# ROCm/k8s-device-plugin

Measured on AMD Instinct MI355X. Metric: pod_admission_device_grants_per_s, higher is better.
Workload: dtype n/a; 1 GPU; model=stub-kubelet-pod-admission, devices_per_allocate=1, parallelism=node-local, server=native, sysfs=live, advertised_gpus=1, present_gpus=1, pinned_cpus=16

## Files before the change

### k8s_device_plugin_amd/native/fastserver.cpp

```cpp

#include <arpa/inet.h>
#include <errno.h>
#include <fcntl.h>
#include <poll.h>
#include <string.h>
#include <sys/socket.h>
#include <sys/un.h>
#include <unistd.h>

#include <algorithm>
#include <atomic>
#include <chrono>
#include <cstdint>
#include <map>
#include <memory>
#include <mutex>
#include <string>
#include <thread>
#include <unordered_map>
#include <vector>

#include <pybind11/pybind11.h>
#include <pybind11/stl.h>

#include "nghttp2_abi.h"
#include "pref_alloc.h"

namespace py = pybind11;
using prefalloc::AllocState;
using prefalloc::preferred_alloc;

namespace {


void put_varint(std::string &out, uint64_t v) {
    while (v >= 0x80) {
        out.push_back((char)(v | 0x80));
        v >>= 7;
    }
    out.push_back((char)v);
}

bool get_varint(const uint8_t *&p, const uint8_t *end, uint64_t &v) {
    v = 0;
    int shift = 0;
    while (p < end && shift < 64) {
        uint8_t b = *p++;
        v |= (uint64_t)(b & 0x7F) << shift;
        if (!(b & 0x80)) return true;
        shift += 7;
    }
    return false;
}

void put_len_delim(std::string &out, int field, const std::string &bytes) {
    put_varint(out, (uint64_t)(field << 3) | 2);
    put_varint(out, bytes.size());
    out += bytes;
}

template <typename F>
bool for_each_field(const uint8_t *p, const uint8_t *end, F cb) {
    while (p < end) {
        uint64_t key;
        if (!get_varint(p, end, key)) return false;
        int field = (int)(key >> 3), wt = (int)(key & 7);
        if (wt == 0) {
            uint64_t v;
            if (!get_varint(p, end, v)) return false;
            cb(field, wt, (const uint8_t *)nullptr, v);
        } else if (wt == 2) {
            uint64_t len;
            if (!get_varint(p, end, len)) return false;
            if ((uint64_t)(end - p) < len) return false;
            cb(field, wt, p, len);
            p += len;
        } else if (wt == 5) {
            if (end - p < 4) return false;
            p += 4;
        } else if (wt == 1) {
            if (end - p < 8) return false;
            p += 8;
        } else {
            return false;
        }
    }
    return true;
}


std::string grpc_frame(const std::string &msg) {
    std::string out;
    out.reserve(msg.size() + 5);
    out.push_back('\0');
    uint32_t n = htonl((uint32_t)msg.size());
    out.append((const char *)&n, 4);
    out += msg;
    return out;
}


struct Conn;

struct Stream {
    std::string path;
    std::string req_body;
    std::string out;
    size_t out_off = 0;
    bool is_listwatch = false;
    bool trailer_sent = false;
    std::string grpc_status = "0";
    std::string grpc_message;
    Conn *conn = nullptr;
};

class Server;

struct Conn {
    int fd = -1;
    nghttp2_session *session = nullptr;
    std::map<int32_t, std::unique_ptr<Stream>> streams;
    std::string wbuf;
    Server *srv = nullptr;
    bool dead = false;
};

class Server {
  public:
    explicit Server(std::string socket_path) : path_(std::move(socket_path)) {}
    ~Server() { stop(); }

    void set_options_response(py::bytes b) {
        std::lock_guard<std::mutex> g(mu_);
        options_ = std::string(b);
    }
    void set_kfd_spec(py::bytes b) {
        std::lock_guard<std::mutex> g(mu_);
        kfd_spec_ = std::string(b);
    }
    void set_device_specs(const std::map<std::string, py::bytes> &specs) {
        std::lock_guard<std::mutex> g(mu_);
        dev_specs_.clear();
        for (auto &kv : specs) dev_specs_[kv.first] = std::string(kv.second);
    }
    void set_list_response(py::bytes b) {
        std::lock_guard<std::mutex> g(mu_);
        list_bytes_ = std::string(b);
    }
    void push_list_update(py::bytes b) {
        {
            std::lock_guard<std::mutex> g(mu_);
            list_bytes_ = std::string(b);
            pending_push_ = true;
        }
        wake();
    }
    void set_prestart_paths(const std::map<std::string, std::string> &paths) {
        std::lock_guard<std::mutex> g(mu_);
        prestart_paths_.clear();
        for (auto &kv : paths) prestart_paths_[kv.first] = kv.second;
    }

    py::dict stats() {
        py::dict d;
        d["allocate_total"] = (uint64_t)n_allocate_.load();
        d["preferred_allocation_total"] = (uint64_t)n_preferred_.load();
        d["list_and_watch_streams_total"] = (uint64_t)n_listwatch_.load();
        d["options_total"] = (uint64_t)n_options_.load();
        d["prestart_total"] = (uint64_t)n_prestart_.load();
        d["unknown_method_total"] = (uint64_t)n_unknown_.load();
        d["list_pushes_total"] = (uint64_t)n_pushes_.load();
        d["connections_total"] = (uint64_t)n_conns_.load();
        d["allocate_handler_ns_total"] = (uint64_t)allocate_ns_.load();
        d["preferred_handler_ns_total"] = (uint64_t)preferred_ns_.load();
        return d;
    }

    void set_allocator_state(
        const std::vector<std::pair<std::string, std::vector<int>>> &groups,
        const std::map<std::string, int> &node_of_id,
        const std::vector<std::tuple<int, int, int>> &weights) {
        std::lock_guard<std::mutex> g(mu_);
        alloc_.load(groups, node_of_id, weights);
    }

    void start() {
        if (running_.exchange(true)) return;
        ::unlink(path_.c_str());
        listen_fd_ = ::socket(AF_UNIX, SOCK_STREAM | SOCK_NONBLOCK, 0);
        if (listen_fd_ < 0) throw std::runtime_error("socket() failed");
        sockaddr_un addr{};
        addr.sun_family = AF_UNIX;
        if (path_.size() >= sizeof(addr.sun_path))
            throw std::runtime_error("socket path too long");
        strncpy(addr.sun_path, path_.c_str(), sizeof(addr.sun_path) - 1);
        if (::bind(listen_fd_, (sockaddr *)&addr, sizeof(addr)) != 0)
            throw std::runtime_error("bind() failed: " +
                                     std::string(strerror(errno)));
        if (::listen(listen_fd_, 16) != 0)
            throw std::runtime_error("listen() failed");
        if (::pipe2(wake_pipe_, O_NONBLOCK) != 0)
            throw std::runtime_error("pipe2() failed");
        loop_ = std::thread([this] { run_loop(); });
    }

    void stop() {
        if (!running_.exchange(false)) return;
        wake();
        if (loop_.joinable()) loop_.join();
        for (auto &c : conns_) destroy_conn(c.get());
        conns_.clear();
        if (listen_fd_ >= 0) ::close(listen_fd_);
        ::close(wake_pipe_[0]);
        ::close(wake_pipe_[1]);
        listen_fd_ = -1;
        ::unlink(path_.c_str());
    }

  private:

    static int on_begin_headers(nghttp2_session *, const nghttp2_frame *frame,
                                void *user) {
        auto *conn = static_cast<Conn *>(user);
        if (frame->hd.type == NGHTTP2_FRAME_HEADERS) {
            auto st = std::make_unique<Stream>();
            st->conn = conn;
            conn->streams[frame->hd.stream_id] = std::move(st);
        }
        return 0;
    }

    static int on_header(nghttp2_session *, const nghttp2_frame *frame,
                         const uint8_t *name, size_t namelen,
                         const uint8_t *value, size_t valuelen, uint8_t,
                         void *user) {
        auto *conn = static_cast<Conn *>(user);
        auto it = conn->streams.find(frame->hd.stream_id);
        if (it == conn->streams.end()) return 0;
        if (namelen == 5 && memcmp(name, ":path", 5) == 0)
            it->second->path.assign((const char *)value, valuelen);
        return 0;
    }

    static int on_data_chunk(nghttp2_session *, uint8_t, int32_t stream_id,
                             const uint8_t *data, size_t len, void *user) {
        auto *conn = static_cast<Conn *>(user);
        auto it = conn->streams.find(stream_id);
        if (it != conn->streams.end())
            it->second->req_body.append((const char *)data, len);
        return 0;
    }

    static int on_frame_recv(nghttp2_session *, const nghttp2_frame *frame,
                             void *user) {
        auto *conn = static_cast<Conn *>(user);
        if ((frame->hd.type == NGHTTP2_FRAME_HEADERS ||
             frame->hd.type == NGHTTP2_FRAME_DATA) &&
            (frame->hd.flags & NGHTTP2_FLAG_END_STREAM)) {
            auto it = conn->streams.find(frame->hd.stream_id);
            if (it != conn->streams.end())
                conn->srv->dispatch(conn, frame->hd.stream_id,
                                    it->second.get());
        }
        return 0;
    }

    static int on_stream_close(nghttp2_session *, int32_t stream_id, uint32_t,
                               void *user) {
        auto *conn = static_cast<Conn *>(user);
        conn->streams.erase(stream_id);
        return 0;
    }

    static ssize_t data_read(nghttp2_session *, int32_t stream_id, uint8_t *buf,
                             size_t length, uint32_t *data_flags,
                             nghttp2_data_source *source, void *user) {
        auto *conn = static_cast<Conn *>(user);
        auto *st = static_cast<Stream *>(source->ptr);
        auto &ng = NgHttp2::get();
        size_t avail;
        {
            std::lock_guard<std::mutex> g(conn->srv->mu_);
            avail = st->out.size() - st->out_off;
            if (avail == 0 && st->is_listwatch) return NGHTTP2_ERR_DEFERRED;
            size_t n = std::min(avail, length);
            memcpy(buf, st->out.data() + st->out_off, n);
            st->out_off += n;
            avail -= n;
            if (st->is_listwatch) {
                if (st->out_off == st->out.size()) {
                    st->out.clear();
                    st->out_off = 0;
                }
                return (ssize_t)n;
            }
            if (avail == 0) {
                *data_flags |= NGHTTP2_DATA_FLAG_EOF | NGHTTP2_DATA_FLAG_NO_END_STREAM;
                if (!st->trailer_sent) {
                    st->trailer_sent = true;
                    nghttp2_nv tr[2];
                    static const char kStatus[] = "grpc-status";
                    static const char kMsg[] = "grpc-message";
                    tr[0] = {(uint8_t *)kStatus, (uint8_t *)st->grpc_status.data(),
                             sizeof(kStatus) - 1, st->grpc_status.size(),
                             NGHTTP2_NV_FLAG_NONE};
                    size_t ntr = 1;
                    if (!st->grpc_message.empty()) {
                        tr[1] = {(uint8_t *)kMsg,
                                 (uint8_t *)st->grpc_message.data(),
                                 sizeof(kMsg) - 1, st->grpc_message.size(),
                                 NGHTTP2_NV_FLAG_NONE};
                        ntr = 2;
                    }
                    ng.submit_trailer(conn->session, stream_id, tr, ntr);
                }
            }
            return (ssize_t)n;
        }
    }


    void dispatch(Conn *conn, int32_t stream_id, Stream *st) {
        std::string msg;
        if (!st->req_body.empty()) {
            if (st->req_body.size() < 5)
                return submit_error(conn, stream_id, st, "13",
                                    "malformed grpc frame: short prefix");
            uint8_t compressed = (uint8_t)st->req_body[0];
            uint32_t len;
            memcpy(&len, st->req_body.data() + 1, 4);
            len = ntohl(len);
            if (compressed != 0)
                return submit_error(conn, stream_id, st, "12",
                                    "grpc message compression not supported");
            if (st->req_body.size() < (size_t)5 + len)
                return submit_error(conn, stream_id, st, "13",
                                    "malformed grpc frame: truncated body");
            msg = st->req_body.substr(5, len);
        }

        const std::string &p = st->path;
        std::string resp;
        if (p == "/v1beta1.DevicePlugin/GetDevicePluginOptions") {
            n_options_.fetch_add(1, std::memory_order_relaxed);
            std::lock_guard<std::mutex> g(mu_);
            resp = options_;
        } else if (p == "/v1beta1.DevicePlugin/PreStartContainer") {
            n_prestart_.fetch_add(1, std::memory_order_relaxed);
            std::string bad;
            if (!handle_prestart(msg, bad))
                return submit_error(
                    conn, stream_id, st, "9",
                    "device " + bad + " failed the pre-start probe");
        } else if (p == "/v1beta1.DevicePlugin/Allocate") {
            n_allocate_.fetch_add(1, std::memory_order_relaxed);
            auto t0 = std::chrono::steady_clock::now();
            resp = handle_allocate(msg);
            allocate_ns_.fetch_add(
                (uint64_t)std::chrono::duration_cast<std::chrono::nanoseconds>(
                    std::chrono::steady_clock::now() - t0).count(),
                std::memory_order_relaxed);
        } else if (p == "/v1beta1.DevicePlugin/GetPreferredAllocation") {
            n_preferred_.fetch_add(1, std::memory_order_relaxed);
            auto t0 = std::chrono::steady_clock::now();
            std::string err;
            bool ok = handle_preferred(msg, resp, err);
            preferred_ns_.fetch_add(
                (uint64_t)std::chrono::duration_cast<std::chrono::nanoseconds>(
                    std::chrono::steady_clock::now() - t0).count(),
                std::memory_order_relaxed);
            if (!ok)
                return submit_error(conn, stream_id, st, "3", err);
        } else if (p == "/v1beta1.DevicePlugin/ListAndWatch") {
            n_listwatch_.fetch_add(1, std::memory_order_relaxed);
            st->is_listwatch = true;
            {
                std::lock_guard<std::mutex> g(mu_);
                st->out = grpc_frame(list_bytes_);
                st->out_off = 0;
            }
            submit_headers_common(conn, stream_id, st);
            return;
        } else {
            n_unknown_.fetch_add(1, std::memory_order_relaxed);
            return submit_error(conn, stream_id, st, "12", "");
        }
        submit_unary(conn, stream_id, st, resp, true);
    }

    void submit_error(Conn *conn, int32_t stream_id, Stream *st,
                      const char *status, const std::string &message) {
        st->grpc_status = status;
        st->grpc_message = message;
        submit_unary(conn, stream_id, st, "", false);
    }

    void submit_headers_common(Conn *conn, int32_t stream_id, Stream *st) {
        auto &ng = NgHttp2::get();
        static const char kS[] = ":status", k200[] = "200";
        static const char kCT[] = "content-type", kGrpc[] = "application/grpc";
        nghttp2_nv hdrs[2] = {
            {(uint8_t *)kS, (uint8_t *)k200, sizeof(kS) - 1, sizeof(k200) - 1,
             NGHTTP2_NV_FLAG_NONE},
            {(uint8_t *)kCT, (uint8_t *)kGrpc, sizeof(kCT) - 1,
             sizeof(kGrpc) - 1, NGHTTP2_NV_FLAG_NONE},
        };
        nghttp2_data_provider prov;
        prov.source.ptr = st;
        prov.read_callback = data_read;
        ng.submit_response(conn->session, stream_id, hdrs, 2, &prov);
    }

    void submit_unary(Conn *conn, int32_t stream_id, Stream *st,
                      const std::string &msg, bool with_body) {
        {
            std::lock_guard<std::mutex> g(mu_);
            st->out = with_body ? grpc_frame(msg) : std::string();
            st->out_off = 0;
        }
        submit_headers_common(conn, stream_id, st);
    }

    bool handle_prestart(const std::string &msg, std::string &bad) {
        std::unordered_map<std::string, std::string> paths;
        {
            std::lock_guard<std::mutex> g(mu_);
            if (prestart_paths_.empty()) return true;
            paths = prestart_paths_;
        }
        bool ok = true;
        const uint8_t *p = (const uint8_t *)msg.data();
        for_each_field(p, p + msg.size(), [&](int field, int wt,
                                              const uint8_t *data,
                                              uint64_t len) {
            if (!ok || field != 1 || wt != 2) return;
            std::string id((const char *)data, len);
            auto it = paths.find(id);
            if (it == paths.end()) return;
            int fd = ::open(it->second.c_str(), O_RDWR | O_CLOEXEC);
            if (fd < 0) {
                ok = false;
                bad = id;
            } else {
                ::close(fd);
            }
        });
        return ok;
    }

    std::string handle_allocate(const std::string &msg) {
        std::lock_guard<std::mutex> g(mu_);
        std::string resp;
        const uint8_t *p = (const uint8_t *)msg.data();
        for_each_field(p, p + msg.size(), [&](int field, int wt,
                                              const uint8_t *data,
                                              uint64_t len) {
            if (field != 1 || wt != 2) return;
            std::string car = kfd_spec_;
            for_each_field(data, data + len, [&](int f2, int wt2,
                                                 const uint8_t *d2,
                                                 uint64_t l2) {
                if (f2 != 1 || wt2 != 2) return;
                std::string id((const char *)d2, l2);
                auto it = dev_specs_.find(id);
                if (it != dev_specs_.end()) car += it->second;
            });
            put_len_delim(resp, 1, car);
        });
        return resp;
    }

    bool handle_preferred(const std::string &msg, std::string &resp,
                          std::string &err) {
        std::lock_guard<std::mutex> g(mu_);
        bool ok = true;
        const uint8_t *p = (const uint8_t *)msg.data();
        for_each_field(p, p + msg.size(), [&](int field, int wt,
                                              const uint8_t *data,
                                              uint64_t len) {
            if (!ok || field != 1 || wt != 2) return;
            std::vector<std::string> available, required;
            int size = 0;
            for_each_field(data, data + len, [&](int f2, int wt2,
                                                 const uint8_t *d2,
                                                 uint64_t l2) {
                if (f2 == 1 && wt2 == 2)
                    available.emplace_back((const char *)d2, l2);
                else if (f2 == 2 && wt2 == 2)
                    required.emplace_back((const char *)d2, l2);
                else if (f2 == 3 && wt2 == 0)
                    size = (int)l2;
            });
            std::vector<std::string> chosen;
            if (!preferred_alloc(alloc_, available, required, size, chosen,
                                 err)) {
                ok = false;
                return;
            }
            std::string car;
            for (auto &id : chosen) put_len_delim(car, 1, id);
            put_len_delim(resp, 1, car);
        });
        return ok;
    }


    void wake() {
        char c = 1;
        ssize_t rc = ::write(wake_pipe_[1], &c, 1);
        (void)rc;
    }

    static constexpr size_t kMaxConns = 256;

    void accept_conn() {
        for (;;) {
            int fd = ::accept4(listen_fd_, nullptr, nullptr, SOCK_NONBLOCK);
            if (fd < 0) return;
            if (conns_.size() >= kMaxConns) {
                ::close(fd);
                continue;
            }
            auto &ng = NgHttp2::get();
            nghttp2_session_callbacks *cbs;
            ng.session_callbacks_new(&cbs);
            ng.set_on_begin_headers(cbs, on_begin_headers);
            ng.set_on_header(cbs, on_header);
            ng.set_on_data_chunk_recv(cbs, on_data_chunk);
            ng.set_on_frame_recv(cbs, on_frame_recv);
            ng.set_on_stream_close(cbs, on_stream_close);
            auto conn = std::make_unique<Conn>();
            conn->fd = fd;
            conn->srv = this;
            ng.session_server_new(&conn->session, cbs, conn.get());
            ng.session_callbacks_del(cbs);
            nghttp2_settings_entry st[1] = {
                {NGHTTP2_SETTINGS_MAX_CONCURRENT_STREAMS, 128}};
            ng.submit_settings(conn->session, NGHTTP2_FLAG_NONE, st, 1);
            n_conns_.fetch_add(1, std::memory_order_relaxed);
            conns_.push_back(std::move(conn));
        }
    }

    void destroy_conn(Conn *c) {
        auto &ng = NgHttp2::get();
        if (c->session) ng.session_del(c->session);
        if (c->fd >= 0) ::close(c->fd);
        c->session = nullptr;
        c->fd = -1;
        c->dead = true;
    }

    bool flush_conn(Conn *c) {
        auto &ng = NgHttp2::get();
        while (!c->wbuf.empty()) {
            ssize_t n = ::write(c->fd, c->wbuf.data(), c->wbuf.size());
            if (n < 0) {
                if (errno == EAGAIN || errno == EWOULDBLOCK) return true;
                return false;
            }
            c->wbuf.erase(0, (size_t)n);
        }
        for (;;) {
            const uint8_t *data = nullptr;
            ssize_t len = ng.session_mem_send(c->session, &data);
            if (len < 0) return false;
            if (len == 0) break;
            ssize_t off = 0;
            while (off < len) {
                ssize_t n = ::write(c->fd, data + off, (size_t)(len - off));
                if (n < 0) {
                    if (errno == EAGAIN || errno == EWOULDBLOCK) {
                        c->wbuf.assign((const char *)data + off,
                                       (size_t)(len - off));
                        return true;
                    }
                    return false;
                }
                off += n;
            }
        }
        return true;
    }

    void run_loop() {
        auto &ng = NgHttp2::get();
        std::vector<pollfd> pfds;
        uint8_t buf[65536];
        while (running_.load()) {
            pfds.clear();
            pfds.push_back({listen_fd_, POLLIN, 0});
            pfds.push_back({wake_pipe_[0], POLLIN, 0});
            for (auto &c : conns_) {
                short ev = POLLIN;
                if (!c->wbuf.empty() || ng.session_want_write(c->session))
                    ev |= POLLOUT;
                pfds.push_back({c->fd, ev, 0});
            }
            int rc = ::poll(pfds.data(), pfds.size(), 500);
            if (rc < 0 && errno != EINTR) break;
            if (!running_.load()) break;

            if (pfds[1].revents & POLLIN) {
                char tmp[64];
                while (::read(wake_pipe_[0], tmp, sizeof(tmp)) > 0) {
                }
                bool do_push;
                std::string bytes;
                {
                    std::lock_guard<std::mutex> g(mu_);
                    do_push = pending_push_;
                    pending_push_ = false;
                    bytes = list_bytes_;
                }
                if (do_push) {
                    n_pushes_.fetch_add(1, std::memory_order_relaxed);
                    std::string framed = grpc_frame(bytes);
                    for (auto &c : conns_) {
                        for (auto &skv : c->streams) {
                            Stream *st = skv.second.get();
                            if (!st->is_listwatch) continue;
                            {
                                std::lock_guard<std::mutex> g(mu_);
                                st->out += framed;
                            }
                            ng.session_resume_data(c->session, skv.first);
                        }
                    }
                }
            }

            if (pfds[0].revents & POLLIN) accept_conn();

            size_t pi = 2;
            for (auto &c : conns_) {
                short rev = pi < pfds.size() ? pfds[pi].revents : 0;
                ++pi;
                if (c->dead) continue;
                if (rev & (POLLERR | POLLHUP)) {
                    destroy_conn(c.get());
                    continue;
                }
                if (rev & POLLIN) {
                    for (;;) {
                        ssize_t n = ::read(c->fd, buf, sizeof(buf));
                        if (n > 0) {
                            if (ng.session_mem_recv(c->session, buf,
                                                    (size_t)n) < 0) {
                                destroy_conn(c.get());
                                break;
                            }
                        } else if (n == 0) {
                            destroy_conn(c.get());
                            break;
                        } else {
                            if (errno != EAGAIN && errno != EWOULDBLOCK)
                                destroy_conn(c.get());
                            break;
                        }
                    }
                }
                if (!c->dead && !flush_conn(c.get()))
                    destroy_conn(c.get());
            }
            conns_.erase(std::remove_if(conns_.begin(), conns_.end(),
                                        [](auto &c) { return c->dead; }),
                         conns_.end());
        }
    }

    std::string path_;
    int listen_fd_ = -1;
    int wake_pipe_[2] = {-1, -1};
    std::thread loop_;
    std::atomic<bool> running_{false};
    std::vector<std::unique_ptr<Conn>> conns_;

    std::atomic<uint64_t> allocate_ns_{0}, preferred_ns_{0};
    std::atomic<uint64_t> n_allocate_{0}, n_preferred_{0}, n_listwatch_{0},
        n_options_{0}, n_prestart_{0}, n_unknown_{0}, n_pushes_{0},
        n_conns_{0};

    std::mutex mu_;
    std::string options_, kfd_spec_, list_bytes_;
    std::unordered_map<std::string, std::string> dev_specs_;
    std::unordered_map<std::string, std::string> prestart_paths_;
    AllocState alloc_;
    bool pending_push_ = false;
};

}

PYBIND11_MODULE(_fastserver, m) {
    m.doc() = "native DevicePlugin v1beta1 gRPC server (nghttp2 over UDS)";
    py::class_<Server>(m, "Server")
        .def(py::init<std::string>())
        .def("set_options_response", &Server::set_options_response)
        .def("set_kfd_spec", &Server::set_kfd_spec)
        .def("set_device_specs", &Server::set_device_specs)
        .def("set_list_response", &Server::set_list_response)
        .def("push_list_update", &Server::push_list_update)
        .def("set_allocator_state", &Server::set_allocator_state)
        .def("stats", &Server::stats)
        .def("set_prestart_paths", &Server::set_prestart_paths)
        .def("start", &Server::start,
             py::call_guard<py::gil_scoped_release>())
        .def("stop", &Server::stop, py::call_guard<py::gil_scoped_release>());
}
```

### k8s_device_plugin_amd/native/pref_alloc.h

```cpp
#pragma once

#include <algorithm>
#include <cstdint>
#include <map>
#include <set>
#include <string>
#include <tuple>
#include <unordered_map>
#include <utility>
#include <vector>

namespace prefalloc {

struct AllocState {
    std::unordered_map<std::string, int> node_of_id;
    std::unordered_map<int, std::string> id_of_node;
    std::vector<std::pair<std::string, std::vector<int>>> groups;
    std::unordered_map<uint64_t, int> weights;
    bool ready = false;

    bool uniform = false;
    std::vector<std::vector<long>> gw;
    std::unordered_map<int, int> group_of_node;

    static uint64_t pair_key(int a, int b) {
        if (a > b) std::swap(a, b);
        return ((uint64_t)(uint32_t)a << 32) | (uint32_t)b;
    }

    int weight(int a, int b) const {
        auto it = weights.find(pair_key(a, b));
        return it == weights.end() ? 0 : it->second;
    }

    void load(const std::vector<std::pair<std::string, std::vector<int>>> &groups_in,
              const std::map<std::string, int> &node_of_id_in,
              const std::vector<std::tuple<int, int, int>> &weights_in) {
        groups = groups_in;
        node_of_id.clear();
        id_of_node.clear();
        for (auto &kv : node_of_id_in) {
            node_of_id[kv.first] = kv.second;
            id_of_node[kv.second] = kv.first;
        }
        weights.clear();
        for (auto &t : weights_in)
            weights[pair_key(std::get<0>(t), std::get<1>(t))] = std::get<2>(t);
        ready = !groups.empty();
        build_uniform_table();
    }

    void build_uniform_table() {
        size_t G = groups.size();
        group_of_node.clear();
        for (size_t g = 0; g < G; ++g)
            for (int n : groups[g].second) group_of_node[n] = (int)g;
        gw.assign(G, std::vector<long>(G, 0));
        uniform = true;
        for (size_t a = 0; a < G && uniform; ++a) {
            for (size_t b = a; b < G && uniform; ++b) {
                bool first = true;
                long w0 = 0;
                for (int i : groups[a].second) {
                    for (int j : groups[b].second) {
                        if (a == b && i >= j) continue;
                        long w = weight(i, j);
                        if (first) { w0 = w; first = false; }
                        else if (w != w0) { uniform = false; break; }
                    }
                    if (!uniform) break;
                }
                gw[a][b] = gw[b][a] = w0;
            }
        }
    }
};

struct Request {
    const AllocState &st;
    std::vector<std::pair<std::string, std::vector<int>>> groups;
    std::vector<int> req_nodes;
    int new_size = 0;
};

template <typename Extra>
struct State {
    uint64_t parents = 0;
    long weight = 0;
    int size = 0;
    uint8_t norder = 0;
    uint8_t order[64];
    Extra x;
};

template <typename S, typename F>
void for_each_node(const Request &rq, const S &s, F fn) {
    int remaining = s.size;
    for (int oi = 0; oi < s.norder; ++oi) {
        const auto &g = rq.groups[s.order[oi]].second;
        int take = std::min((int)g.size(), remaining);
        for (int i = 0; i < take; ++i) fn(g[i]);
        remaining -= take;
    }
}

struct UniformScorer {
    struct Extra { long rowsum[64]; };
    using S = State<Extra>;
    const Request &rq;
    const size_t n_orig;
    std::vector<int> orig_of;

    explicit UniformScorer(const Request &r)
        : rq(r), n_orig(r.st.groups.size()), orig_of(r.groups.size()) {
        for (size_t i = 0; i < rq.groups.size(); ++i)
            orig_of[i] = rq.st.group_of_node.at(rq.groups[i].second[0]);
    }
    void add_row(S &s, int b, long m) const {
        for (size_t h = 0; h < n_orig; ++h) s.x.rowsum[h] += m * rq.st.gw[b][h];
    }
    void add_group(S &s, size_t fidx, int m) const {
        int b = orig_of[fidx];
        s.weight += (long)m * s.x.rowsum[b] +
                    (long)m * (m - 1) / 2 * rq.st.gw[b][b];
        add_row(s, b, m);
    }
    void add_required(S &s) const {
        for (int rn : rq.req_nodes) {
            int b = rq.st.group_of_node.at(rn);
            s.weight += s.x.rowsum[b];
            add_row(s, b, 1);
        }
    }
};

struct PerNodeScorer {
    struct Extra {};
    using S = State<Extra>;
    const Request &rq;
    std::vector<int> nodes;

    explicit PerNodeScorer(const Request &r) : rq(r) {}
    void add_node(S &s, int n) {
        for (int o : nodes) s.weight += rq.st.weight(o, n);
        nodes.push_back(n);
    }
    void add_group(S &s, size_t fidx, int m) {
        nodes.clear();
        for_each_node(rq, s, [&](int n) { nodes.push_back(n); });
        for (int i = 0; i < m; ++i) add_node(s, rq.groups[fidx].second[i]);
    }
    void add_required(S &s) {
        nodes.clear();
        for_each_node(rq, s, [&](int n) { nodes.push_back(n); });
        for (int rn : rq.req_nodes) add_node(s, rn);
    }
};

template <typename Scorer>
bool search(const Request &rq, Scorer sc, std::vector<int> &out) {
    using S = typename Scorer::S;
    const size_t G = rq.groups.size();
    std::vector<S> queue;
    queue.reserve(G <= 16 ? (1u << G) : 4096);
    std::vector<bool> seen_bm;
    std::set<uint64_t> seen_set;
    const bool use_bm = G <= 20;
    if (use_bm) seen_bm.assign(1u << G, false);
    auto seen_test_set = [&](uint64_t p) {
        if (use_bm) {
            if (seen_bm[p]) return true;
            seen_bm[p] = true;
            return false;
        }
        return !seen_set.insert(p).second;
    };
    S best{};
    bool have_best = false;
    auto extend = [&](S s, size_t idx) {
        int take = std::min((int)rq.groups[idx].second.size(),
                            rq.new_size - s.size);
        sc.add_group(s, idx, take);
        s.parents |= 1ull << idx;
        s.order[s.norder++] = (uint8_t)idx;
        s.size += take;
        if (s.size == rq.new_size) {
            sc.add_required(s);
            if (!have_best || s.weight < best.weight) {
                best = s;
                have_best = true;
            }
        } else if (!seen_test_set(s.parents)) {
            queue.push_back(s);
        }
    };
    for (size_t idx = 0; idx < G; ++idx) extend(S{}, idx);
    for (size_t qi = 0; qi < queue.size(); ++qi) {
        const S cur = queue[qi];
        if (__builtin_popcountll(cur.parents) == (int)G) continue;
        for (size_t idx = 0; idx < G; ++idx)
            if (!(cur.parents & (1ull << idx))) extend(cur, idx);
    }
    if (!have_best) return false;
    for_each_node(rq, best, [&](int n) { out.push_back(n); });
    out.insert(out.end(), rq.req_nodes.begin(), rq.req_nodes.end());
    return true;
}

inline bool preferred_alloc(const AllocState &st,
                            const std::vector<std::string> &available,
                            const std::vector<std::string> &required, int size,
                            std::vector<std::string> &out, std::string &err) {
    if (!st.ready) { err = "allocator not initialized"; return false; }
    if (size <= 0) { err = "allocation size must be a positive integer"; return false; }
    if ((int)available.size() < size) { err = "available devices count less than allocation size"; return false; }
    if ((int)required.size() > size) { err = "must-include set larger than allocation size"; return false; }
    if (required.size() > available.size()) { err = "must-include set larger than available set"; return false; }
    if ((int)available.size() == size) { out = available; return true; }
    if ((int)required.size() == size) { out = required; return true; }
    std::set<std::string> avail_set(available.begin(), available.end());
    for (auto &r : required)
        if (!avail_set.count(r)) { err = "must-include devices not all available"; return false; }

    Request rq{st, {}, {}, 0};
    std::set<int> avail_nodes, req_nodes;
    for (auto &a : available) {
        auto it = st.node_of_id.find(a);
        if (it != st.node_of_id.end()) avail_nodes.insert(it->second);
    }
    for (auto &r : required) {
        auto it = st.node_of_id.find(r);
        if (it != st.node_of_id.end()) {
            req_nodes.insert(it->second);
            rq.req_nodes.push_back(it->second);
        }
    }

    for (auto &g : st.groups) {
        std::vector<int> ids;
        for (int n : g.second)
            if (avail_nodes.count(n) && !req_nodes.count(n)) ids.push_back(n);
        if (!ids.empty()) rq.groups.emplace_back(g.first, std::move(ids));
    }
    std::stable_sort(rq.groups.begin(), rq.groups.end(),
                     [](auto &a, auto &b) {
                         if (a.second.size() != b.second.size())
                             return a.second.size() < b.second.size();
                         return a.first < b.first;
                     });
    if (rq.groups.size() > 64) { err = "too many device groups"; return false; }
    rq.new_size = size - (int)rq.req_nodes.size();

    const bool closed_form = st.uniform && st.groups.size() <= 64;
    std::vector<int> nodes;
    if (!(closed_form ? search(rq, UniformScorer(rq), nodes)
                      : search(rq, PerNodeScorer(rq), nodes))) {
        err = "no candidate subset found";
        return false;
    }
    for (int n : nodes) {
        auto it = st.id_of_node.find(n);
        if (it == st.id_of_node.end()) continue;
        if (!closed_form && !avail_set.count(it->second)) continue;
        out.push_back(it->second);
    }
    return true;
}

}
```

### k8s_device_plugin_amd/plugin/metrics.py

```python

from __future__ import annotations

import logging
from typing import Optional

log = logging.getLogger(__name__)

_COUNTER_HELP = {
    "allocate_total": "Allocate RPCs served",
    "allocate_handler_ns_total": "cumulative Allocate handler time (ns)",
    "preferred_handler_ns_total": "cumulative GetPreferredAllocation handler time (ns)",
    "preferred_allocation_total": "GetPreferredAllocation RPCs served",
    "list_and_watch_streams_total": "ListAndWatch streams opened",
    "options_total": "GetDevicePluginOptions RPCs served",
    "prestart_total": "PreStartContainer RPCs served",
    "unknown_method_total": "RPCs to unknown methods",
    "list_pushes_total": "device-list updates pushed to streams",
    "connections_total": "kubelet connections accepted",
}


class _ManagerCollector:

    def __init__(self, manager):
        self.manager = manager

    def collect(self):
        from prometheus_client.core import CounterMetricFamily, GaugeMetricFamily

        g = GaugeMetricFamily(
            "amdgpu_dp_advertised_devices",
            "devices advertised per resource",
            labels=["resource"],
        )
        for resource, inst in self.manager.plugins.items():
            g.add_metric([resource], len(inst.plugin.devices))
        yield g

        df = GaugeMetricFamily(
            "amdgpu_dp_deep_probe_failed_gpus",
            "physical GPUs currently pinned Unhealthy by the deep probe",
            labels=["resource"],
        )
        for resource, inst in self.manager.plugins.items():
            df.add_metric([resource], len(inst.plugin._deep_failed))
        yield df

        bs = GaugeMetricFamily(
            "amdgpu_dp_deep_probe_bad_simds",
            "SIMDs that failed the last deep-probe CU sweep, summed over "
            "GPUs (0 while the sweep is off)",
            labels=["resource"],
        )
        for resource, inst in self.manager.plugins.items():
            bs.add_metric([resource],
                          sum(inst.plugin._sweep_bad_simds.values()))
        yield bs

        counters = {}
        for resource, inst in self.manager.plugins.items():
            if inst.native:
                try:
                    stats = inst.server._srv.stats()
                except Exception:
                    continue
                for key, value in stats.items():
                    counters.setdefault(key, []).append((resource, value))
        for key, entries in counters.items():
            c = CounterMetricFamily(
                f"amdgpu_dp_{key}",
                _COUNTER_HELP.get(key, key),
                labels=["resource"],
            )
            for resource, value in entries:
                c.add_metric([resource], value)
            yield c


def start_metrics_server(manager, port: int) -> Optional[object]:
    if port <= 0:
        return None
    try:
        import prometheus_client
        from prometheus_client.core import CollectorRegistry
    except ImportError:
        log.warning("prometheus_client not installed; metrics disabled")
        return None

    registry = CollectorRegistry()
    registry.register(_ManagerCollector(manager))
    prometheus_client.start_http_server(port, registry=registry)
    log.info("metrics endpoint on :%d/metrics", port)
    return registry
```

Baseline: 14370 device-grants/s.

## Cut per-RPC copies, batch socket writes, and densify preferred-allocation tables

The dispatcher now parses request bodies in place rather than copying them out, and builds responses with the gRPC prefix reserved up front so framing happens in place. Allocate and preferred-allocation handlers reuse scratch buffers held by the server. The allocator drops std::set and hash-map lookups in favour of dense index tables and a flat group-weight matrix. The flush path gathers nghttp2 output into one buffer of up to 64 KiB per write() and the read loop stops after a short read; new read/write counters are exported. The workload is one device per Allocate, so the preferred-allocation rework may matter little, while the syscall batching and fewer copies target per-RPC overhead.

```diff
diff --git a/k8s_device_plugin_amd/native/fastserver.cpp b/k8s_device_plugin_amd/native/fastserver.cpp
--- a/k8s_device_plugin_amd/native/fastserver.cpp
+++ b/k8s_device_plugin_amd/native/fastserver.cpp
@@ -89,14 +89,22 @@
 }
 
 
+constexpr size_t kGrpcPrefix = 5;
+
 std::string grpc_frame(const std::string &msg) {
     std::string out;
-    out.reserve(msg.size() + 5);
+    out.reserve(msg.size() + kGrpcPrefix);
     out.push_back('\0');
     uint32_t n = htonl((uint32_t)msg.size());
     out.append((const char *)&n, 4);
     out += msg;
     return out;
+}
+
+void grpc_frame_in_place(std::string &framed) {
+    framed[0] = '\0';
+    uint32_t n = htonl((uint32_t)(framed.size() - kGrpcPrefix));
+    memcpy(&framed[1], &n, 4);
 }
 
 
@@ -121,6 +129,8 @@
     nghttp2_session *session = nullptr;
     std::map<int32_t, std::unique_ptr<Stream>> streams;
     std::string wbuf;
+    size_t woff = 0;
+    bool want_out() const { return woff < wbuf.size(); }
     Server *srv = nullptr;
     bool dead = false;
 };
@@ -173,6 +183,9 @@
         d["connections_total"] = (uint64_t)n_conns_.load();
         d["allocate_handler_ns_total"] = (uint64_t)allocate_ns_.load();
         d["preferred_handler_ns_total"] = (uint64_t)preferred_ns_.load();
+        d["socket_writes_total"] = (uint64_t)n_writes_.load();
+        d["socket_reads_total"] = (uint64_t)n_reads_.load();
+        d["socket_write_would_block_total"] = (uint64_t)n_would_block_.load();
         return d;
     }
 
@@ -321,7 +334,8 @@
 
 
     void dispatch(Conn *conn, int32_t stream_id, Stream *st) {
-        std::string msg;
+        const uint8_t *msg = nullptr;
+        size_t msg_len = 0;
         if (!st->req_body.empty()) {
             if (st->req_body.size() < 5)
                 return submit_error(conn, stream_id, st, "13",
@@ -336,26 +350,27 @@
             if (st->req_body.size() < (size_t)5 + len)
                 return submit_error(conn, stream_id, st, "13",
                                     "malformed grpc frame: truncated body");
-            msg = st->req_body.substr(5, len);
+            msg = (const uint8_t *)st->req_body.data() + 5;
+            msg_len = len;
         }
 
         const std::string &p = st->path;
-        std::string resp;
+        std::string resp(kGrpcPrefix, '\0');
         if (p == "/v1beta1.DevicePlugin/GetDevicePluginOptions") {
             n_options_.fetch_add(1, std::memory_order_relaxed);
             std::lock_guard<std::mutex> g(mu_);
-            resp = options_;
+            resp += options_;
         } else if (p == "/v1beta1.DevicePlugin/PreStartContainer") {
             n_prestart_.fetch_add(1, std::memory_order_relaxed);
             std::string bad;
-            if (!handle_prestart(msg, bad))
+            if (!handle_prestart(msg, msg_len, bad))
                 return submit_error(
                     conn, stream_id, st, "9",
                     "device " + bad + " failed the pre-start probe");
         } else if (p == "/v1beta1.DevicePlugin/Allocate") {
             n_allocate_.fetch_add(1, std::memory_order_relaxed);
             auto t0 = std::chrono::steady_clock::now();
-            resp = handle_allocate(msg);
+            handle_allocate(msg, msg_len, resp);
             allocate_ns_.fetch_add(
                 (uint64_t)std::chrono::duration_cast<std::chrono::nanoseconds>(
                     std::chrono::steady_clock::now() - t0).count(),
@@ -364,7 +379,7 @@
             n_preferred_.fetch_add(1, std::memory_order_relaxed);
             auto t0 = std::chrono::steady_clock::now();
             std::string err;
-            bool ok = handle_preferred(msg, resp, err);
+            bool ok = handle_preferred(msg, msg_len, resp, err);
             preferred_ns_.fetch_add(
                 (uint64_t)std::chrono::duration_cast<std::chrono::nanoseconds>(
                     std::chrono::steady_clock::now() - t0).count(),
@@ -385,14 +400,14 @@
             n_unknown_.fetch_add(1, std::memory_order_relaxed);
             return submit_error(conn, stream_id, st, "12", "");
         }
-        submit_unary(conn, stream_id, st, resp, true);
+        submit_unary(conn, stream_id, st, std::move(resp));
     }
 
     void submit_error(Conn *conn, int32_t stream_id, Stream *st,
                       const char *status, const std::string &message) {
         st->grpc_status = status;
         st->grpc_message = message;
-        submit_unary(conn, stream_id, st, "", false);
+        submit_unary(conn, stream_id, st, std::string());
     }
 
     void submit_headers_common(Conn *conn, int32_t stream_id, Stream *st) {
@@ -412,16 +427,17 @@
     }
 
     void submit_unary(Conn *conn, int32_t stream_id, Stream *st,
-                      const std::string &msg, bool with_body) {
+                      std::string &&framed) {
+        if (!framed.empty()) grpc_frame_in_place(framed);
         {
             std::lock_guard<std::mutex> g(mu_);
-            st->out = with_body ? grpc_frame(msg) : std::string();
+            st->out = std::move(framed);
             st->out_off = 0;
         }
         submit_headers_common(conn, stream_id, st);
     }
 
-    bool handle_prestart(const std::string &msg, std::string &bad) {
+    bool handle_prestart(const uint8_t *p, size_t msg_len, std::string &bad) {
         std::unordered_map<std::string, std::string> paths;
         {
             std::lock_guard<std::mutex> g(mu_);
@@ -429,10 +445,9 @@
             paths = prestart_paths_;
         }
         bool ok = true;
-        const uint8_t *p = (const uint8_t *)msg.data();
-        for_each_field(p, p + msg.size(), [&](int field, int wt,
-                                              const uint8_t *data,
-                                              uint64_t len) {
+        for_each_field(p, p + msg_len, [&](int field, int wt,
+                                           const uint8_t *data,
+                                           uint64_t len) {
             if (!ok || field != 1 || wt != 2) return;
             std::string id((const char *)data, len);
             auto it = paths.find(id);
@@ -448,15 +463,14 @@
         return ok;
     }
 
-    std::string handle_allocate(const std::string &msg) {
+    void handle_allocate(const uint8_t *p, size_t msg_len, std::string &resp) {
         std::lock_guard<std::mutex> g(mu_);
-        std::string resp;
-        const uint8_t *p = (const uint8_t *)msg.data();
-        for_each_field(p, p + msg.size(), [&](int field, int wt,
-                                              const uint8_t *data,
-                                              uint64_t len) {
+        std::string &car = car_;
+        for_each_field(p, p + msg_len, [&](int field, int wt,
+                                           const uint8_t *data,
+                                           uint64_t len) {
             if (field != 1 || wt != 2) return;
-            std::string car = kfd_spec_;
+            car = kfd_spec_;
             for_each_field(data, data + len, [&](int f2, int wt2,
                                                  const uint8_t *d2,
                                                  uint64_t l2) {
@@ -467,19 +481,23 @@
             });
             put_len_delim(resp, 1, car);
         });
-        return resp;
-    }
-
-    bool handle_preferred(const std::string &msg, std::string &resp,
+    }
+
+    bool handle_preferred(const uint8_t *p, size_t msg_len, std::string &resp,
                           std::string &err) {
         std::lock_guard<std::mutex> g(mu_);
         bool ok = true;
-        const uint8_t *p = (const uint8_t *)msg.data();
-        for_each_field(p, p + msg.size(), [&](int field, int wt,
-                                              const uint8_t *data,
-                                              uint64_t len) {
+        std::vector<std::string> &available = pref_available_,
+                                 &required = pref_required_,
+                                 &chosen = pref_chosen_;
+        std::string &car = car_;
+        for_each_field(p, p + msg_len, [&](int field, int wt,
+                                           const uint8_t *data,
+                                           uint64_t len) {
             if (!ok || field != 1 || wt != 2) return;
-            std::vector<std::string> available, required;
+            available.clear();
+            required.clear();
+            chosen.clear();
             int size = 0;
             for_each_field(data, data + len, [&](int f2, int wt2,
                                                  const uint8_t *d2,
@@ -491,13 +509,12 @@
                 else if (f2 == 3 && wt2 == 0)
                     size = (int)l2;
             });
-            std::vector<std::string> chosen;
-            if (!preferred_alloc(alloc_, available, required, size, chosen,
-                                 err)) {
+            if (!preferred_alloc(alloc_, scratch_, available, required, size,
+                                 chosen, err)) {
                 ok = false;
                 return;
             }
-            std::string car;
+            car.clear();
             for (auto &id : chosen) put_len_delim(car, 1, id);
             put_len_delim(resp, 1, car);
         });
@@ -551,36 +568,43 @@
         c->dead = true;
     }
 
+    static constexpr size_t kGatherLimit = 65536;
+
     bool flush_conn(Conn *c) {
         auto &ng = NgHttp2::get();
-        while (!c->wbuf.empty()) {
-            ssize_t n = ::write(c->fd, c->wbuf.data(), c->wbuf.size());
+        for (;;) {
+            if (!c->want_out()) {
+                c->wbuf.clear();
+                c->woff = 0;
+            } else if (c->woff >= kGatherLimit) {
+                c->wbuf.erase(0, c->woff);
+                c->woff = 0;
+            }
+            while (c->wbuf.size() - c->woff < kGatherLimit) {
+                const uint8_t *data = nullptr;
+                ssize_t len = ng.session_mem_send(c->session, &data);
+                if (len < 0) return false;
+                if (len == 0) break;
+                c->wbuf.append((const char *)data, (size_t)len);
+            }
+            if (!c->want_out()) return true;
+            size_t want = c->wbuf.size() - c->woff;
+            ssize_t n = ::write(c->fd, c->wbuf.data() + c->woff, want);
+            n_writes_.fetch_add(1, std::memory_order_relaxed);
             if (n < 0) {
-                if (errno == EAGAIN || errno == EWOULDBLOCK) return true;
+                if (errno == EINTR) continue;
+                if (errno == EAGAIN || errno == EWOULDBLOCK) {
+                    n_would_block_.fetch_add(1, std::memory_order_relaxed);
+                    return true;
+                }
                 return false;
             }
-            c->wbuf.erase(0, (size_t)n);
-        }
-        for (;;) {
-            const uint8_t *data = nullptr;
-            ssize_t len = ng.session_mem_send(c->session, &data);
-            if (len < 0) return false;
-            if (len == 0) break;
-            ssize_t off = 0;
-            while (off < len) {
-                ssize_t n = ::write(c->fd, data + off, (size_t)(len - off));
-                if (n < 0) {
-                    if (errno == EAGAIN || errno == EWOULDBLOCK) {
-                        c->wbuf.assign((const char *)data + off,
-                                       (size_t)(len - off));
-                        return true;
-                    }
-                    return false;
-                }
-                off += n;
-            }
-        }
-        return true;
+            c->woff += (size_t)n;
+            if ((size_t)n < want) {
+                n_would_block_.fetch_add(1, std::memory_order_relaxed);
+                return true;
+            }
+        }
     }
 
     void run_loop() {
@@ -593,7 +617,7 @@
             pfds.push_back({wake_pipe_[0], POLLIN, 0});
             for (auto &c : conns_) {
                 short ev = POLLIN;
-                if (!c->wbuf.empty() || ng.session_want_write(c->session))
+                if (c->want_out() || ng.session_want_write(c->session))
                     ev |= POLLOUT;
                 pfds.push_back({c->fd, ev, 0});
             }
@@ -644,12 +668,14 @@
                 if (rev & POLLIN) {
                     for (;;) {
                         ssize_t n = ::read(c->fd, buf, sizeof(buf));
+                        n_reads_.fetch_add(1, std::memory_order_relaxed);
                         if (n > 0) {
                             if (ng.session_mem_recv(c->session, buf,
                                                     (size_t)n) < 0) {
                                 destroy_conn(c.get());
                                 break;
                             }
+                            if ((size_t)n < sizeof(buf)) break;
                         } else if (n == 0) {
                             destroy_conn(c.get());
                             break;
@@ -679,13 +705,16 @@
     std::atomic<uint64_t> allocate_ns_{0}, preferred_ns_{0};
     std::atomic<uint64_t> n_allocate_{0}, n_preferred_{0}, n_listwatch_{0},
         n_options_{0}, n_prestart_{0}, n_unknown_{0}, n_pushes_{0},
-        n_conns_{0};
+        n_conns_{0}, n_writes_{0}, n_reads_{0}, n_would_block_{0};
 
     std::mutex mu_;
     std::string options_, kfd_spec_, list_bytes_;
     std::unordered_map<std::string, std::string> dev_specs_;
     std::unordered_map<std::string, std::string> prestart_paths_;
     AllocState alloc_;
+    prefalloc::Scratch scratch_;
+    std::vector<std::string> pref_available_, pref_required_, pref_chosen_;
+    std::string car_;
     bool pending_push_ = false;
 };
 
diff --git a/k8s_device_plugin_amd/native/pref_alloc.h b/k8s_device_plugin_amd/native/pref_alloc.h
--- a/k8s_device_plugin_amd/native/pref_alloc.h
+++ b/k8s_device_plugin_amd/native/pref_alloc.h
@@ -3,7 +3,6 @@
 #include <algorithm>
 #include <cstdint>
 #include <map>
-#include <set>
 #include <string>
 #include <tuple>
 #include <unordered_map>
@@ -13,15 +12,24 @@
 namespace prefalloc {
 
 struct AllocState {
-    std::unordered_map<std::string, int> node_of_id;
-    std::unordered_map<int, std::string> id_of_node;
     std::vector<std::pair<std::string, std::vector<int>>> groups;
     std::unordered_map<uint64_t, int> weights;
     bool ready = false;
 
     bool uniform = false;
-    std::vector<std::vector<long>> gw;
-    std::unordered_map<int, int> group_of_node;
+    std::vector<long> gw;
+
+    std::vector<int> node_ids;
+    std::unordered_map<std::string, int> id_index;
+    std::vector<std::string> ids;
+    std::vector<int> node_of_idx;
+    std::vector<int> id_of_dense;
+    std::vector<int> group_of_dense;
+    std::vector<int> member_begin;
+    std::vector<int> members;
+    std::vector<int> parent_rank;
+    static constexpr size_t kDenseWeightNodes = 256;
+    std::vector<int> wdense;
 
     static uint64_t pair_key(int a, int b) {
         if (a > b) std::swap(a, b);
@@ -31,31 +39,33 @@
     int weight(int a, int b) const {
         auto it = weights.find(pair_key(a, b));
         return it == weights.end() ? 0 : it->second;
+    }
+
+    int dense_weight(int a, int b) const {
+        if (!wdense.empty()) return wdense[(size_t)a * node_ids.size() + b];
+        return weight(node_ids[a], node_ids[b]);
+    }
+
+    int dense_of(int node) const {
+        return (int)(std::lower_bound(node_ids.begin(), node_ids.end(), node) -
+                     node_ids.begin());
     }
 
     void load(const std::vector<std::pair<std::string, std::vector<int>>> &groups_in,
               const std::map<std::string, int> &node_of_id_in,
               const std::vector<std::tuple<int, int, int>> &weights_in) {
         groups = groups_in;
-        node_of_id.clear();
-        id_of_node.clear();
-        for (auto &kv : node_of_id_in) {
-            node_of_id[kv.first] = kv.second;
-            id_of_node[kv.second] = kv.first;
-        }
         weights.clear();
         for (auto &t : weights_in)
             weights[pair_key(std::get<0>(t), std::get<1>(t))] = std::get<2>(t);
         ready = !groups.empty();
         build_uniform_table();
+        build_request_tables(node_of_id_in);
     }
 
     void build_uniform_table() {
         size_t G = groups.size();
-        group_of_node.clear();
-        for (size_t g = 0; g < G; ++g)
-            for (int n : groups[g].second) group_of_node[n] = (int)g;
-        gw.assign(G, std::vector<long>(G, 0));
+        gw.assign(G * G, 0);
         uniform = true;
         for (size_t a = 0; a < G && uniform; ++a) {
             for (size_t b = a; b < G && uniform; ++b) {
@@ -70,144 +80,282 @@
                     }
                     if (!uniform) break;
                 }
-                gw[a][b] = gw[b][a] = w0;
+                gw[a * G + b] = gw[b * G + a] = w0;
             }
         }
     }
+
+    void build_request_tables(const std::map<std::string, int> &node_of_id_in) {
+        const size_t G = groups.size();
+        node_ids.clear();
+        for (auto &g : groups)
+            node_ids.insert(node_ids.end(), g.second.begin(), g.second.end());
+        for (auto &kv : node_of_id_in) node_ids.push_back(kv.second);
+        std::sort(node_ids.begin(), node_ids.end());
+        node_ids.erase(std::unique(node_ids.begin(), node_ids.end()),
+                       node_ids.end());
+        const size_t N = node_ids.size();
+
+        id_index.clear();
+        ids.clear();
+        node_of_idx.clear();
+        id_of_dense.assign(N, -1);
+        for (auto &kv : node_of_id_in) {
+            int idx = (int)ids.size();
+            id_index[kv.first] = idx;
+            ids.push_back(kv.first);
+            node_of_idx.push_back(dense_of(kv.second));
+            id_of_dense[node_of_idx.back()] = idx;
+        }
+        group_of_dense.assign(N, -1);
+        member_begin.assign(1, 0);
+        members.clear();
+        for (size_t g = 0; g < G; ++g) {
+            for (int n : groups[g].second) {
+                members.push_back(dense_of(n));
+                group_of_dense[members.back()] = (int)g;
+            }
+            member_begin.push_back((int)members.size());
+        }
+
+        std::vector<int> by_key(G);
+        for (size_t g = 0; g < G; ++g) by_key[g] = (int)g;
+        std::sort(by_key.begin(), by_key.end(), [&](int a, int b) {
+            return groups[a].first < groups[b].first;
+        });
+        parent_rank.assign(G, 0);
+        for (size_t i = 1; i < G; ++i)
+            parent_rank[by_key[i]] =
+                parent_rank[by_key[i - 1]] +
+                (groups[by_key[i - 1]].first != groups[by_key[i]].first);
+
+        wdense.clear();
+        if (N <= kDenseWeightNodes) {
+            wdense.assign(N * N, 0);
+            for (size_t a = 0; a < N; ++a)
+                for (size_t b = 0; b < N; ++b)
+                    wdense[a * N + b] = weight(node_ids[a], node_ids[b]);
+        }
+    }
+};
+
+struct SearchState {
+    uint64_t parents;
+    long weight;
+    int size;
+    int pred;
+    int group;
+};
+
+struct Scratch {
+    std::vector<uint8_t> avail_id, avail_node, req_node;
+    std::vector<int> req_nodes;
+    std::vector<int> fg_nodes;
+    struct Filtered { int begin, len, orig; };
+    std::vector<Filtered> fg;
+    std::vector<SearchState> states;
+    std::vector<long> rows, row_tmp;
+    std::vector<uint64_t> seen_bits;
+    std::vector<uint64_t> seen_hash;
+    size_t seen_hash_used = 0;
+    std::vector<int> nodes;
+    std::vector<int> result;
 };
 
 struct Request {
     const AllocState &st;
-    std::vector<std::pair<std::string, std::vector<int>>> groups;
-    std::vector<int> req_nodes;
+    Scratch &sc;
     int new_size = 0;
 };
 
-template <typename Extra>
-struct State {
-    uint64_t parents = 0;
-    long weight = 0;
-    int size = 0;
-    uint8_t norder = 0;
-    uint8_t order[64];
-    Extra x;
-};
-
-template <typename S, typename F>
-void for_each_node(const Request &rq, const S &s, F fn) {
-    int remaining = s.size;
-    for (int oi = 0; oi < s.norder; ++oi) {
-        const auto &g = rq.groups[s.order[oi]].second;
-        int take = std::min((int)g.size(), remaining);
-        for (int i = 0; i < take; ++i) fn(g[i]);
+struct SeenSet {
+    Scratch &sc;
+    const bool use_bits;
+
+    SeenSet(Scratch &s, size_t G) : sc(s), use_bits(G <= 20) {
+        if (use_bits) {
+            size_t words = ((size_t(1) << G) + 63) / 64;
+            if (sc.seen_bits.size() < words) sc.seen_bits.resize(words, 0);
+        } else if (sc.seen_hash.empty()) {
+            sc.seen_hash.assign(1024, 0);
+        }
+    }
+    static size_t slot_of(uint64_t p, size_t mask) {
+        return (size_t)((p * 0x9E3779B97F4A7C15ull) >> 20) & mask;
+    }
+    bool test_set(uint64_t p) {
+        if (use_bits) {
+            uint64_t &w = sc.seen_bits[p >> 6], bit = 1ull << (p & 63);
+            if (w & bit) return true;
+            w |= bit;
+            return false;
+        }
+        if ((sc.seen_hash_used + 1) * 2 > sc.seen_hash.size()) grow();
+        size_t mask = sc.seen_hash.size() - 1;
+        for (size_t i = slot_of(p, mask);; i = (i + 1) & mask) {
+            if (sc.seen_hash[i] == p) return true;
+            if (sc.seen_hash[i] == 0) {
+                sc.seen_hash[i] = p;
+                ++sc.seen_hash_used;
+                return false;
+            }
+        }
+    }
+    void grow() {
+        std::vector<uint64_t> old(sc.seen_hash.size() * 2, 0);
+        old.swap(sc.seen_hash);
+        size_t mask = sc.seen_hash.size() - 1;
+        for (uint64_t p : old) {
+            if (!p) continue;
+            size_t i = slot_of(p, mask);
+            while (sc.seen_hash[i]) i = (i + 1) & mask;
+            sc.seen_hash[i] = p;
+        }
+    }
+    void clear() {
+        if (use_bits) {
+            for (size_t i = 1; i < sc.states.size(); ++i)
+                sc.seen_bits[sc.states[i].parents >> 6] = 0;
+        } else if (sc.seen_hash_used * 8 > sc.seen_hash.size()) {
+            std::fill(sc.seen_hash.begin(), sc.seen_hash.end(), 0);
+            sc.seen_hash_used = 0;
+        } else {
+            size_t mask = sc.seen_hash.size() - 1;
+            for (size_t s = 1; s < sc.states.size(); ++s)
+                for (size_t i = slot_of(sc.states[s].parents, mask);
+                     sc.seen_hash[i]; i = (i + 1) & mask)
+                    sc.seen_hash[i] = 0;
+            sc.seen_hash_used = 0;
+        }
+    }
+};
+
+template <typename F>
+void for_each_node(const Request &rq, int pred, int last, int size, F fn) {
+    int chain[65], n = 0;
+    if (last >= 0) chain[n++] = last;
+    for (int s = pred; s > 0; s = rq.sc.states[s].pred)
+        chain[n++] = rq.sc.states[s].group;
+    int remaining = size;
+    while (n-- > 0) {
+        const Scratch::Filtered &g = rq.sc.fg[chain[n]];
+        int take = std::min(g.len, remaining);
+        for (int i = 0; i < take; ++i) fn(rq.sc.fg_nodes[g.begin + i]);
         remaining -= take;
     }
 }
 
+
 struct UniformScorer {
-    struct Extra { long rowsum[64]; };
-    using S = State<Extra>;
     const Request &rq;
-    const size_t n_orig;
-    std::vector<int> orig_of;
+    const size_t stride;
+    const long *gw;
 
     explicit UniformScorer(const Request &r)
-        : rq(r), n_orig(r.st.groups.size()), orig_of(r.groups.size()) {
-        for (size_t i = 0; i < rq.groups.size(); ++i)
-            orig_of[i] = rq.st.group_of_node.at(rq.groups[i].second[0]);
-    }
-    void add_row(S &s, int b, long m) const {
-        for (size_t h = 0; h < n_orig; ++h) s.x.rowsum[h] += m * rq.st.gw[b][h];
-    }
-    void add_group(S &s, size_t fidx, int m) const {
-        int b = orig_of[fidx];
-        s.weight += (long)m * s.x.rowsum[b] +
-                    (long)m * (m - 1) / 2 * rq.st.gw[b][b];
-        add_row(s, b, m);
-    }
-    void add_required(S &s) const {
-        for (int rn : rq.req_nodes) {
-            int b = rq.st.group_of_node.at(rn);
-            s.weight += s.x.rowsum[b];
-            add_row(s, b, 1);
-        }
+        : rq(r), stride(r.st.groups.size()), gw(r.st.gw.data()) {
+        rq.sc.rows.assign(stride, 0);
+        rq.sc.row_tmp.resize(stride);
+    }
+    long add_group(int pred, int fidx, int m) const {
+        int b = rq.sc.fg[fidx].orig;
+        return rq.sc.states[pred].weight +
+               (long)m * rq.sc.rows[pred * stride + b] +
+               (long)m * (m - 1) / 2 * gw[b * stride + b];
+    }
+    void queued(int pred, int fidx, int m) const {
+        int b = rq.sc.fg[fidx].orig;
+        rq.sc.rows.resize(rq.sc.states.size() * stride);
+        const long *src = &rq.sc.rows[pred * stride];
+        long *dst = &rq.sc.rows[(rq.sc.states.size() - 1) * stride];
+        for (size_t h = 0; h < stride; ++h)
+            dst[h] = src[h] + (long)m * gw[b * stride + h];
+    }
+    long add_required(int pred, int fidx, int m, long weight) const {
+        if (rq.sc.req_nodes.empty()) return weight;
+        int b = rq.sc.fg[fidx].orig;
+        const long *src = &rq.sc.rows[pred * stride];
+        long *row = rq.sc.row_tmp.data();
+        for (size_t h = 0; h < stride; ++h)
+            row[h] = src[h] + (long)m * gw[b * stride + h];
+        for (int rn : rq.sc.req_nodes) {
+            int rb = rq.st.group_of_dense[rn];
+            if (rb < 0) continue;
+            weight += row[rb];
+            for (size_t h = 0; h < stride; ++h) row[h] += gw[rb * stride + h];
+        }
+        return weight;
     }
 };
 
 struct PerNodeScorer {
-    struct Extra {};
-    using S = State<Extra>;
     const Request &rq;
-    std::vector<int> nodes;
 
     explicit PerNodeScorer(const Request &r) : rq(r) {}
-    void add_node(S &s, int n) {
-        for (int o : nodes) s.weight += rq.st.weight(o, n);
-        nodes.push_back(n);
-    }
-    void add_group(S &s, size_t fidx, int m) {
-        nodes.clear();
-        for_each_node(rq, s, [&](int n) { nodes.push_back(n); });
-        for (int i = 0; i < m; ++i) add_node(s, rq.groups[fidx].second[i]);
-    }
-    void add_required(S &s) {
-        nodes.clear();
-        for_each_node(rq, s, [&](int n) { nodes.push_back(n); });
-        for (int rn : rq.req_nodes) add_node(s, rn);
+    long add_node(long weight, int n) const {
+        for (int o : rq.sc.nodes) weight += rq.st.dense_weight(o, n);
+        rq.sc.nodes.push_back(n);
+        return weight;
+    }
+    long add_group(int pred, int fidx, int m) const {
+        rq.sc.nodes.clear();
+        for_each_node(rq, pred, -1, rq.sc.states[pred].size,
+                      [&](int n) { rq.sc.nodes.push_back(n); });
+        long weight = rq.sc.states[pred].weight;
+        const Scratch::Filtered &g = rq.sc.fg[fidx];
+        for (int i = 0; i < m; ++i)
+            weight = add_node(weight, rq.sc.fg_nodes[g.begin + i]);
+        return weight;
+    }
+    void queued(int, int, int) const {}
+    long add_required(int, int, int, long weight) const {
+        for (int rn : rq.sc.req_nodes) weight = add_node(weight, rn);
+        return weight;
     }
 };
 
 template <typename Scorer>
-bool search(const Request &rq, Scorer sc, std::vector<int> &out) {
-    using S = typename Scorer::S;
-    const size_t G = rq.groups.size();
-    std::vector<S> queue;
-    queue.reserve(G <= 16 ? (1u << G) : 4096);
-    std::vector<bool> seen_bm;
-    std::set<uint64_t> seen_set;
-    const bool use_bm = G <= 20;
-    if (use_bm) seen_bm.assign(1u << G, false);
-    auto seen_test_set = [&](uint64_t p) {
-        if (use_bm) {
-            if (seen_bm[p]) return true;
-            seen_bm[p] = true;
-            return false;
-        }
-        return !seen_set.insert(p).second;
+bool search(const Request &rq, const Scorer &sc) {
+    Scratch &s = rq.sc;
+    const size_t G = s.fg.size();
+    s.states.clear();
+    s.states.push_back({0, 0, 0, 0, -1});
+    SeenSet seen(s, G);
+    long best_weight = 0;
+    int best_pred = -1, best_group = -1;
+    auto extend = [&](int pred, size_t idx) {
+        const int size = s.states[pred].size;
+        const int take = std::min(s.fg[idx].len, rq.new_size - size);
+        long weight = sc.add_group(pred, (int)idx, take);
+        const uint64_t parents = s.states[pred].parents | (1ull << idx);
+        if (size + take == rq.new_size) {
+            weight = sc.add_required(pred, (int)idx, take, weight);
+            if (best_pred < 0 || weight < best_weight) {
+                best_weight = weight;
+                best_pred = pred;
+                best_group = (int)idx;
+            }
+        } else if (!seen.test_set(parents)) {
+            s.states.push_back({parents, weight, size + take, pred, (int)idx});
+            sc.queued(pred, (int)idx, take);
+        }
     };
-    S best{};
-    bool have_best = false;
-    auto extend = [&](S s, size_t idx) {
-        int take = std::min((int)rq.groups[idx].second.size(),
-                            rq.new_size - s.size);
-        sc.add_group(s, idx, take);
-        s.parents |= 1ull << idx;
-        s.order[s.norder++] = (uint8_t)idx;
-        s.size += take;
-        if (s.size == rq.new_size) {
-            sc.add_required(s);
-            if (!have_best || s.weight < best.weight) {
-                best = s;
-                have_best = true;
-            }
-        } else if (!seen_test_set(s.parents)) {
-            queue.push_back(s);
-        }
-    };
-    for (size_t idx = 0; idx < G; ++idx) extend(S{}, idx);
-    for (size_t qi = 0; qi < queue.size(); ++qi) {
-        const S cur = queue[qi];
-        if (__builtin_popcountll(cur.parents) == (int)G) continue;
+    for (size_t idx = 0; idx < G; ++idx) extend(0, idx);
+    for (size_t qi = 1; qi < s.states.size(); ++qi) {
+        const uint64_t parents = s.states[qi].parents;
+        if (__builtin_popcountll(parents) == (int)G) continue;
         for (size_t idx = 0; idx < G; ++idx)
-            if (!(cur.parents & (1ull << idx))) extend(cur, idx);
-    }
-    if (!have_best) return false;
-    for_each_node(rq, best, [&](int n) { out.push_back(n); });
-    out.insert(out.end(), rq.req_nodes.begin(), rq.req_nodes.end());
+            if (!(parents & (1ull << idx))) extend((int)qi, idx);
+    }
+    seen.clear();
+    if (best_pred < 0) return false;
+    s.result.clear();
+    for_each_node(rq, best_pred, best_group, rq.new_size,
+                  [&](int n) { s.result.push_back(n); });
+    s.result.insert(s.result.end(), s.req_nodes.begin(), s.req_nodes.end());
     return true;
 }
 
-inline bool preferred_alloc(const AllocState &st,
+inline bool preferred_alloc(const AllocState &st, Scratch &sc,
                             const std::vector<std::string> &available,
                             const std::vector<std::string> &required, int size,
                             std::vector<std::string> &out, std::string &err) {
@@ -218,53 +366,84 @@
     if (required.size() > available.size()) { err = "must-include set larger than available set"; return false; }
     if ((int)available.size() == size) { out = available; return true; }
     if ((int)required.size() == size) { out = required; return true; }
-    std::set<std::string> avail_set(available.begin(), available.end());
-    for (auto &r : required)
-        if (!avail_set.count(r)) { err = "must-include devices not all available"; return false; }
-
-    Request rq{st, {}, {}, 0};
-    std::set<int> avail_nodes, req_nodes;
+
+    sc.avail_id.assign(st.ids.size(), 0);
+    sc.avail_node.assign(st.node_ids.size(), 0);
+    sc.req_node.assign(st.node_ids.size(), 0);
+    sc.req_nodes.clear();
     for (auto &a : available) {
-        auto it = st.node_of_id.find(a);
-        if (it != st.node_of_id.end()) avail_nodes.insert(it->second);
+        auto it = st.id_index.find(a);
+        if (it == st.id_index.end()) continue;
+        sc.avail_id[it->second] = 1;
+        sc.avail_node[st.node_of_idx[it->second]] = 1;
     }
     for (auto &r : required) {
-        auto it = st.node_of_id.find(r);
-        if (it != st.node_of_id.end()) {
-            req_nodes.insert(it->second);
-            rq.req_nodes.push_back(it->second);
-        }
-    }
-
-    for (auto &g : st.groups) {
-        std::vector<int> ids;
-        for (int n : g.second)
-            if (avail_nodes.count(n) && !req_nodes.count(n)) ids.push_back(n);
-        if (!ids.empty()) rq.groups.emplace_back(g.first, std::move(ids));
-    }
-    std::stable_sort(rq.groups.begin(), rq.groups.end(),
-                     [](auto &a, auto &b) {
-                         if (a.second.size() != b.second.size())
-                             return a.second.size() < b.second.size();
-                         return a.first < b.first;
-                     });
-    if (rq.groups.size() > 64) { err = "too many device groups"; return false; }
-    rq.new_size = size - (int)rq.req_nodes.size();
-
+        auto it = st.id_index.find(r);
+        if (it != st.id_index.end()
+                ? !sc.avail_id[it->second]
+                : std::find(available.begin(), available.end(), r) ==
+                      available.end()) {
+            err = "must-include devices not all available";
+            return false;
+        }
+    }
+    for (auto &r : required) {
+        auto it = st.id_index.find(r);
+        if (it == st.id_index.end()) continue;
+        int n = st.node_of_idx[it->second];
+        sc.req_node[n] = 1;
+        sc.req_nodes.push_back(n);
+    }
+
+    sc.fg.clear();
+    sc.fg_nodes.clear();
+    for (size_t g = 0; g + 1 < st.member_begin.size(); ++g) {
+        int begin = (int)sc.fg_nodes.size();
+        for (int i = st.member_begin[g]; i < st.member_begin[g + 1]; ++i) {
+            int n = st.members[i];
+            if (sc.avail_node[n] && !sc.req_node[n]) sc.fg_nodes.push_back(n);
+        }
+        int len = (int)sc.fg_nodes.size() - begin;
+        if (len) sc.fg.push_back({begin, len, (int)g});
+    }
+    if (sc.fg.size() > 64) { err = "too many device groups"; return false; }
+    for (size_t i = 1; i < sc.fg.size(); ++i) {
+        Scratch::Filtered f = sc.fg[i];
+        size_t j = i;
+        for (; j > 0; --j) {
+            const Scratch::Filtered &p = sc.fg[j - 1];
+            bool less = f.len != p.len
+                            ? f.len < p.len
+                            : st.parent_rank[f.orig] < st.parent_rank[p.orig];
+            if (!less) break;
+            sc.fg[j] = p;
+        }
+        sc.fg[j] = f;
+    }
+    for (auto &f : sc.fg) f.orig = st.group_of_dense[sc.fg_nodes[f.begin]];
+
+    Request rq{st, sc, size - (int)sc.req_nodes.size()};
     const bool closed_form = st.uniform && st.groups.size() <= 64;
-    std::vector<int> nodes;
-    if (!(closed_form ? search(rq, UniformScorer(rq), nodes)
-                      : search(rq, PerNodeScorer(rq), nodes))) {
+    if (!(closed_form ? search(rq, UniformScorer(rq))
+                      : search(rq, PerNodeScorer(rq)))) {
         err = "no candidate subset found";
         return false;
     }
-    for (int n : nodes) {
-        auto it = st.id_of_node.find(n);
-        if (it == st.id_of_node.end()) continue;
-        if (!closed_form && !avail_set.count(it->second)) continue;
-        out.push_back(it->second);
+    for (int n : sc.result) {
+        int idx = st.id_of_dense[n];
+        if (idx < 0) continue;
+        if (!closed_form && !sc.avail_id[idx]) continue;
+        out.push_back(st.ids[idx]);
     }
     return true;
 }
 
+inline bool preferred_alloc(const AllocState &st,
+                            const std::vector<std::string> &available,
+                            const std::vector<std::string> &required, int size,
+                            std::vector<std::string> &out, std::string &err) {
+    Scratch sc;
+    return preferred_alloc(st, sc, available, required, size, out, err);
 }
+
+}
diff --git a/k8s_device_plugin_amd/plugin/metrics.py b/k8s_device_plugin_amd/plugin/metrics.py
--- a/k8s_device_plugin_amd/plugin/metrics.py
+++ b/k8s_device_plugin_amd/plugin/metrics.py
@@ -17,6 +17,11 @@
     "unknown_method_total": "RPCs to unknown methods",
     "list_pushes_total": "device-list updates pushed to streams",
     "connections_total": "kubelet connections accepted",
+    "socket_writes_total": "write() calls on kubelet connections",
+    "socket_reads_total": "read() calls on kubelet connections",
+    "socket_write_would_block_total": (
+        "writes the socket took none or only part of (back-pressure)"
+    ),
 }
 
 
```

Result: faster. 15630 device-grants/s (median of 6 runs) (+8.7%).
